# latteine1217/NSFnet

Hardware: AMD Instinct MI355X
Metric: collocation-pt NS-residual evals/sec, Re=2000 6x256 MLP (higher is better)
Workload: dtype bf16x3 (bf16 MFMA, hi/lo split, f32 accumulate)

## Files before the change

include/nsfnet_pinn.h:

```cpp
#ifndef NSFNET_PINN_H
#define NSFNET_PINN_H

#include <stdint.h>

#ifdef __cplusplus
extern "C" {
#endif

typedef struct pinn_net_s* pinn_net_t;
typedef struct pinn_plan_s* pinn_plan_t;

enum {
  PINN_FLD_U = 0, PINN_FLD_V, PINN_FLD_UX, PINN_FLD_UY, PINN_FLD_VX, PINN_FLD_VY,
  PINN_FLD_EQ1, PINN_FLD_EQ2, PINN_FLD_EQ3, PINN_FLD_EQ4, PINN_FLD_P, PINN_FLD_COUNT
};
#define PINN_NLOSS 8

const char* pinn_last_error(void);
int pinn_abi_version(void);

int pinn_net_create(int n_out, int n_hidden_layers, int hidden, pinn_net_t* out);
int pinn_net_destroy(pinn_net_t net);
int pinn_net_set_precision(pinn_net_t net, int prec_fwd, int prec_bwd, int prec_dw);
int64_t pinn_net_num_params(pinn_net_t net);
int64_t pinn_net_prep_floats(pinn_net_t net);
int pinn_net_prepare(pinn_net_t net, const float* params, float* prep, void* stream);

int pinn_plan_create(pinn_net_t net, int64_t n_points, int streams, pinn_plan_t* out);
int pinn_plan_destroy(pinn_plan_t plan);
int64_t pinn_plan_padded_points(pinn_plan_t plan);
int64_t pinn_plan_workspace_bytes(pinn_plan_t plan, int with_backward);
const char* pinn_plan_kernel(pinn_plan_t plan, int which);

int pinn_residual_forward(pinn_plan_t plan, void* ws, const float* prep,
                          const float* x, const float* y, const float* e, const float* w,
                          float* vis_t_minus, float* vis_t_out, float* fields,
                          float Re, float vis_t0, float alpha_evm, float coord_scale,
                          int save, float* loss_sums, void* stream);

int pinn_residual_backward(pinn_plan_t plan, void* ws, const float* prep,
                           const float* x, const float* y, const float* e, const float* w,
                           const float* vis_t, const float* fields, const float* coef_eq4,
                           float Re, float coord_scale, float* ebar_out, void* stream);

int pinn_residual_backward_phases(pinn_plan_t plan, void* ws, const float* prep,
                                  const float* x, const float* y, const float* e, const float* w,
                                  const float* vis_t, const float* fields, const float* coef_eq4,
                                  float Re, float coord_scale, float* ebar_out, int phases, void* stream);

int pinn_residual_forward_backward(pinn_plan_t plan, void* ws, const float* prep,
                                   const float* x, const float* y, const float* e, const float* w,
                                   float* vis_t_minus, float* vis_t_out, float* fields,
                                   const float* coef_eq4, float Re, float vis_t0, float alpha_evm,
                                   float coord_scale, float* loss_sums, float* ebar_out, void* stream);

// ... 94 lines not shown
```

nsfnet_amd/_lib.py:

```python
import ctypes
import os

_HERE = os.path.dirname(os.path.abspath(__file__))
LIB_PATH = os.environ.get("NSFNET_PINN_LIB") or os.path.join(_HERE, "lib", "libnsfnet_pinn.so")

c_void_p, c_int, c_int64, c_float, c_double = ctypes.c_void_p, ctypes.c_int, ctypes.c_int64, ctypes.c_float, ctypes.c_double

SIGNATURES = {
    "pinn_last_error": (ctypes.c_char_p, []),
    "pinn_abi_version": (c_int, []),
    "pinn_net_create": (c_int, [c_int, c_int, c_int, ctypes.POINTER(c_void_p)]),
    "pinn_net_destroy": (c_int, [c_void_p]),
    "pinn_net_set_precision": (c_int, [c_void_p, c_int, c_int, c_int]),
    "pinn_net_num_params": (c_int64, [c_void_p]),
    "pinn_net_prep_floats": (c_int64, [c_void_p]),
    "pinn_net_prepare": (c_int, [c_void_p, c_void_p, c_void_p, c_void_p]),
    "pinn_plan_create": (c_int, [c_void_p, c_int64, c_int, ctypes.POINTER(c_void_p)]),
    "pinn_plan_destroy": (c_int, [c_void_p]),
    "pinn_plan_padded_points": (c_int64, [c_void_p]),
    "pinn_plan_workspace_bytes": (c_int64, [c_void_p, c_int]),
    "pinn_plan_kernel": (ctypes.c_char_p, [c_void_p, c_int]),
    "pinn_residual_forward": (c_int, [c_void_p, c_void_p, c_void_p, c_void_p, c_void_p, c_void_p, c_void_p,
                                      c_void_p, c_void_p, c_void_p, c_float, c_float, c_float, c_float,
                                      c_int, c_void_p, c_void_p]),
    "pinn_residual_backward": (c_int, [c_void_p, c_void_p, c_void_p, c_void_p, c_void_p, c_void_p, c_void_p,
                                       c_void_p, c_void_p, ctypes.POINTER(c_float), c_float, c_float,
                                       c_void_p, c_void_p]),
    "pinn_residual_backward_phases": (c_int, [c_void_p, c_void_p, c_void_p, c_void_p, c_void_p, c_void_p, c_void_p,
                                              c_void_p, c_void_p, ctypes.POINTER(c_float), c_float, c_float,
                                              c_void_p, c_int, c_void_p]),
    "pinn_residual_forward_backward": (c_int, [c_void_p, c_void_p, c_void_p, c_void_p, c_void_p, c_void_p, c_void_p,
                                               c_void_p, c_void_p, c_void_p, ctypes.POINTER(c_float), c_float, c_float,
                                               c_float, c_float, c_void_p, c_void_p, c_void_p]),
    "pinn_value_forward": (c_int, [c_void_p, c_void_p, c_void_p, c_void_p, c_void_p,
                                   ctypes.POINTER(c_void_p), ctypes.POINTER(c_void_p), ctypes.POINTER(c_float),
                                   c_int, c_void_p, c_void_p]),
    "pinn_value_backward": (c_int, [c_void_p, c_void_p, c_void_p, c_void_p, c_void_p, c_void_p, c_void_p]),
    "pinn_grad_reduce": (c_int, [c_void_p, c_int, ctypes.POINTER(c_void_p), ctypes.POINTER(c_void_p),
                                 c_void_p, c_int, c_void_p]),
    "pinn_adam_step": (c_int, [c_void_p, c_void_p, c_void_p, c_void_p, c_int64,
                               c_float, c_float, c_float, c_float, c_int64, c_void_p]),
    "pinn_adam_step_dev": (c_int, [c_void_p, c_void_p, c_void_p, c_void_p, c_int64,
                                   c_float, c_float, c_float, c_float, c_void_p, c_void_p]),
    "pinn_resample_scratch_bytes": (c_int64, [c_int64]),
# ... 75 lines not shown
```

nsfnet_amd/build.py:

```python
import os
import subprocess
import sys
from concurrent.futures import ThreadPoolExecutor

HERE = os.path.dirname(os.path.abspath(__file__))
CSRC = os.path.join(HERE, "csrc")
OBJ = os.path.join(CSRC, "build")
LIBDIR = os.path.join(HERE, "lib")
LIB = os.path.join(LIBDIR, "libnsfnet_pinn.so")
SOURCES = ["fwd.hip", "bwd.hip", "dw.hip", "fwd_bf16.hip", "bwd_bf16.hip", "dw_bf16.hip", "fwd_wide.hip", "bwd_wide.hip", "dw_wide.hip",
           "fwd_bf16_wide.hip", "bwd_bf16_wide.hip", "dw_bf16_wide.hip", "fwd_bf16_pipe.hip", "bwd_bf16_pipe.hip", "fwd_bf16_split.hip", "bwd_bf16_split.hip", "fwdbwd_bf16_split.hip", "fwd_bf16_wsplit.hip", "bwd_bf16_wsplit.hip", "misc.hip", "resample.hip", "lbfgs.hip", "balance.hip", "confgrad.hip", "batch.hip", "rba.hip", "optim.hip", "rwf.hip", "capi.hip"]
HEADERS = ["kernels.h", "layout.h", "spill.h", "spill_io.h", "bf16_util.h", "reduce_util.h", "point_stage.h", "split_phases.h", "wsplit_phases.h", "wave8_bodies.h", "optim.h", "rwf.h", "xwg_fold.h", os.path.join("..", "..", "include", "nsfnet_pinn.h")]
FLAGS = ["-O3", "--offload-arch=gfx950", "-fPIC", "-std=c++17", "-Wall", "-Wno-unused-function"]
_PIPE = ["-fno-slp-vectorize", "-mllvm", "-pragma-unroll-threshold=1000000"]
EXTRA_FLAGS = {"fwd_bf16_pipe.hip": _PIPE, "bwd_bf16_pipe.hip": _PIPE, "fwd_bf16_split.hip": _PIPE, "bwd_bf16_split.hip": _PIPE, "fwdbwd_bf16_split.hip": _PIPE,
               "fwd_bf16_wsplit.hip": _PIPE, "bwd_bf16_wsplit.hip": _PIPE}


def _hipcc():
    for cand in (os.environ.get("HIPCC"), "/opt/rocm/bin/hipcc", "hipcc"):
        if cand and (os.path.isabs(cand) and os.path.exists(cand) or not os.path.isabs(cand)):
            return cand
    return "hipcc"


def _stale(target, deps):
    if not os.path.exists(target):
        return True
    t = os.path.getmtime(target)
    return any(os.path.getmtime(d) > t for d in deps)


def build(force=False, verbose=False):
    os.makedirs(OBJ, exist_ok=True)
    os.makedirs(LIBDIR, exist_ok=True)
# ... 35 lines not shown
```

nsfnet_amd/csrc/balance.hip:

```cpp
#include <cmath>

#include "kernels.h"

namespace {

constexpr int kBlk = 64;
constexpr int kUpdThreads = 256;

__device__ __forceinline__ double nmax(double a, double b) { return (b > a || b != b) ? b : a; }

__device__ __forceinline__ void wave_abs_stats(float v, double& mx, double& sm) {
  mx = fabs((double)v); sm = mx;
#pragma unroll
  for (int off = 32; off > 0; off >>= 1) {
    mx = nmax(mx, __shfl_down(mx, off, 64));
    sm = __dadd_rn(sm, __shfl_down(sm, off, 64));
  }
}

__global__ __launch_bounds__(512) void reduce_terms_kernel(TermReduceArgs a) {
  __shared__ double part[3][8][64];
  const int H = a.H, HP = a.HP, L = a.L;
  const size_t P = flat_total(H, L, a.n_out);
  const int lane = threadIdx.x & 63, w = threadIdx.x >> 6;
  const size_t p = blockIdx.x * (size_t)64 + lane;
  const bool live = p < P;
  const ReduceLoc loc = live ? reduce_locate(p, H, HP, L, a.n_out) : ReduceLoc{-1, -1, 0};
  const size_t SG = sg_total(HP, L);
  int k = 0;
  for (int t = 0; t < 3; ++t) {
    double s = 0.0;
    for (int j = 0; j < a.nsrc[t]; ++j, ++k)
      if (live) s = reduce_source_add(s, a.src[k], loc, HP, SG, w);
    part[t][w][lane] = s;
  }
  __syncthreads();
  if (w != 0) return;
  float vt[3];
  for (int t = 0; t < 3; ++t) {
    float v = 0.f;
    if (a.out[t] && live) {
      double s = part[t][0][lane];
#pragma unroll
      for (int i = 1; i < 8; ++i) s += part[t][i][lane];
      v = (a.acc_mask >> t) & 1 ? a.out[t][p] + (float)s : (float)s;
      a.out[t][p] = v;
    }
    if (a.partials) {
      double mx, sm;
      wave_abs_stats(v, mx, sm);
      if (lane == 0) {
        a.partials[(size_t)blockIdx.x * 6 + 2 * t] = mx;
        a.partials[(size_t)blockIdx.x * 6 + 2 * t + 1] = sm;
      }
    }
    vt[t] = v;
  }
  if (a.gram) wave_gram(vt[0], vt[1], vt[2], lane, a.gram + (size_t)blockIdx.x * 6);
}

__global__ __launch_bounds__(64) void balance_stats_kernel(const float* __restrict__ v0, const float* __restrict__ v1,
                                                           const float* __restrict__ v2, long n,
                                                           double* __restrict__ partials) {
  const long p = blockIdx.x * (long)kBlk + threadIdx.x;
  const float* v[3] = {v0, v1, v2};
  for (int t = 0; t < 3; ++t) {
    double mx, sm;
    wave_abs_stats(v[t] && p < n ? v[t][p] : 0.f, mx, sm);
    if (threadIdx.x == 0) {
      partials[(size_t)blockIdx.x * 6 + 2 * t] = mx;
      partials[(size_t)blockIdx.x * 6 + 2 * t + 1] = sm;
    }
  }
}

__global__ __launch_bounds__(kUpdThreads) void balance_update_kernel(const double* __restrict__ partials, long nblk,
                                                                     long n, int terms, double beta,
                                                                     float* __restrict__ lam, double* record) {
  __shared__ double red[kUpdThreads][6];
  const int tid = threadIdx.x;
  double acc[6] = {0, 0, 0, 0, 0, 0};
// ... 40 lines not shown
}

__global__ void balance_combine_kernel(float* g, const float* gr, const float* __restrict__ gb,
                                       const float* __restrict__ gs, const float* __restrict__ lam, long n) {
  const float lb = lam[0], ls = gs ? lam[1] : 0.f;
  for (long i = blockIdx.x * (long)blockDim.x + threadIdx.x; i < n; i += (long)gridDim.x * blockDim.x) {
    float v = fmaf(lb, gb[i], gr[i]);
    if (gs) v = fmaf(ls, gs[i], v);
    g[i] = v;
  }
}

int status() {
  hipError_t e = hipGetLastError();
  return e == hipSuccess ? 0 : -(int)e;
}

}

long balance_blocks(long n) { return (n + kBlk - 1) / kBlk; }

int launch_reduce_terms(const TermReduceArgs& a, hipStream_t s) {
  size_t P = flat_total(a.H, a.L, a.n_out);
  hipLaunchKernelGGL(reduce_terms_kernel, dim3((unsigned)((P + 63) / 64)), dim3(512), 0, s, a);
  return status();
}

int launch_balance_stats(const float* v0, const float* v1, const float* v2, long n, double* partials, hipStream_t s) {
  hipLaunchKernelGGL(balance_stats_kernel, dim3((unsigned)balance_blocks(n)), dim3(kBlk), 0, s, v0, v1, v2, n, partials);
  return status();
}

int launch_balance_update(const double* partials, long n, int terms, double beta, float* lam, double* record,
                          hipStream_t s) {
  hipLaunchKernelGGL(balance_update_kernel, dim3(1), dim3(kUpdThreads), 0, s, partials, balance_blocks(n), n, terms,
                     beta, lam, record);
  return status();
}

int launch_balance_combine(float* g, const float* gr, const float* gb, const float* gs, const float* lam, long n,
                           hipStream_t s) {
  int blocks = (int)((n + 255) / 256);
  if (blocks > 2048) blocks = 2048;
  hipLaunchKernelGGL(balance_combine_kernel, dim3(blocks), dim3(256), 0, s, g, gr, gb, gs, lam, n);
  return status();
}
```

nsfnet_amd/csrc/capi.hip:

```cpp
#include <cmath>
#include <cstdio>
#include <cstring>
#include <cstdlib>
#include <new>

#include "../../include/nsfnet_pinn.h"
#include "kernels.h"
#include "optim.h"
#include "rwf.h"

static_assert((int)PINN_FLD_COUNT == (int)FLD_COUNT, "field plane enum mismatch");

static thread_local char g_err[512] = "";
static int fail(int code, const char* fmt, const char* a = "", long b = 0) {
  snprintf(g_err, sizeof(g_err), fmt, a, b);
  return code;
}
static int hipfail(int rc, const char* what) {
  if (rc == -1000) return fail(-22, "%s: unsupported hidden width or spill layout (code %ld)", what, (long)rc);
  return fail(rc, "%s: HIP error %ld", what, (long)-rc);
}

struct Switches {
  int sched_f, sched_b;
// ... 352 lines not shown
int pinn_plan_create(pinn_net_t net, int64_t n_points, int streams, pinn_plan_t* out) {
  if (!net || !out) return fail(-22, "pinn_plan_create: null argument%s");
  if (streams != 1 && streams != 4) return fail(-22, "pinn_plan_create: streams must be 1 or 4%s");
  if (n_points < 1 || n_points > (int64_t)1 << 30) return fail(-22, "pinn_plan_create: bad point count %s%ld", "", (long)n_points);
  pinn_plan_s* p = new (std::nothrow) pinn_plan_s;
  if (!p) return fail(-12, "pinn_plan_create: out of host memory%s");
  int rc = resolve_plan(p, *net, (long)n_points, streams, num_cus(), read_switches());
  if (rc) { delete p; return rc; }
  int ndev = 0;
  if (hipGetDeviceCount(&ndev) != hipSuccess) { ndev = 0; (void)hipGetLastError(); }
  if (ndev > 0) {
    rc = configure_plan(p);
    if (rc) { delete p; return hipfail(rc, "pinn_plan_create(kernel attributes)"); }
  }
  *out = p;
  return 0;
}
int pinn_plan_destroy(pinn_plan_t plan) { delete plan; return 0; }
int64_t pinn_plan_padded_points(pinn_plan_t plan) { return plan ? plan->npad : -1; }
const char* pinn_plan_kernel(pinn_plan_t plan, int which) {
  if (!plan || which < 0 || which > 2) return nullptr;
  return plan->role[which == 0 ? ROLE_FWD_SAVE : which == 1 ? ROLE_BWD : ROLE_DW].name;
}
int64_t pinn_plan_workspace_bytes(pinn_plan_t plan, int with_backward) {
  if (!plan) return -1;
  return (int64_t)(with_backward ? plan->bytes_all : plan->bytes_fwd);
}

static int run_loss_sums(const Role& r, const FwdArgs& a, float* loss_sums, hipStream_t s, const char* what) {
  if (!loss_sums) return 0;
  int rc = launch_loss_sums(a.partials, r.grid, loss_sums, s);
  return rc ? hipfail(rc, what) : 0;
}

int pinn_residual_forward(pinn_plan_t plan, void* ws, const float* prep,
                          const float* x, const float* y, const float* e, const float* w,
                          float* vis_t_minus, float* vis_t_out, float* fields,
                          float Re, float vis_t0, float alpha_evm, float coord_scale,
                          int save, float* loss_sums, void* stream) {
  if (!plan || !ws || !prep || !x || !y || !fields) return fail(-22, "pinn_residual_forward: null argument%s");
  if (plan->streams != 4) return fail(-22, "pinn_residual_forward: plan is not a residual (4-stream) plan%s");
  if (!(Re > 0.f)) return fail(-22, "pinn_residual_forward: Re must be > 0%s");
  const FwdArgs a = residual_fwd_args(plan, ws, prep, x, y, e, w, vis_t_minus, vis_t_out, fields, Re, vis_t0, alpha_evm,
                                      coord_scale, save, true);
  const Role& r = plan->role[save ? ROLE_FWD_SAVE : ROLE_FWD];
  int rc = run_fwd(plan, r, a, (hipStream_t)stream);
// ... 493 lines not shown
```

nsfnet_amd/csrc/kernels.h:

```cpp
#pragma once
#include <hip/hip_runtime.h>
#include <type_traits>
#include "layout.h"
#include "spill.h"

typedef float f32x16 __attribute__((ext_vector_type(16)));
typedef float f32x4 __attribute__((ext_vector_type(4)));

#ifdef __HIPCC__
typedef __attribute__((address_space(1))) f32x4 gf32x4;
__device__ __forceinline__ gf32x4* pin_base(const void* q) {
  const unsigned long long b = (unsigned long long)q;
  const unsigned lo = __builtin_amdgcn_readfirstlane((unsigned)b), hi = __builtin_amdgcn_readfirstlane((unsigned)(b >> 32));
  return (gf32x4*)(((unsigned long long)hi << 32) | lo);
}
template <typename... Params, typename... Args>
static int launch_or_configure(void (*kernel)(Params...), dim3 grid, dim3 block, size_t lds, hipStream_t s, int configure,
                               const Args&... args) {
  if (configure)
    return -(int)hipFuncSetAttribute(reinterpret_cast<const void*>(kernel), hipFuncAttributeMaxDynamicSharedMemorySize, PINN_LDS_MAX);
  hipLaunchKernelGGL(kernel, grid, block, lds, s, args...);
  return -(int)hipGetLastError();
}
template <class F>
// ... 64 lines not shown

struct ReduceLoc { int sgi; int layer; size_t slab_off; };
__device__ __forceinline__ ReduceLoc reduce_locate(size_t p, int H, int HP, int L, int n_out) {
  ReduceLoc r{-1, -1, 0};
  if (p < (size_t)2 * H) {
    int o = (int)(p / 2), j = (int)(p % 2);
    r.sgi = (j == 0 ? sg_w0x(HP, L) : sg_w0y(HP, L)) + o;
  } else if (p < (size_t)3 * H) {
    r.sgi = sg_db(HP, 0) + (int)(p - 2 * H);
  } else if (p < flat_w(H, L)) {
    size_t rel = p - (size_t)3 * H;
    size_t per = (size_t)H * H + H;
    int l = 1 + (int)(rel / per);
    size_t q = rel % per;
    if (q < (size_t)H * H) { r.layer = l; r.slab_off = (q / H) * HP + (q % H); }
    else r.sgi = sg_db(HP, l) + (int)(q - (size_t)H * H);
  } else {
    size_t q = p - flat_w(H, L);
    if (q < (size_t)n_out * H) r.sgi = sg_wout(HP, L) + (int)(q / H) * HP + (int)(q % H);
    else r.sgi = sg_bout(HP, L) + (int)(q - (size_t)n_out * H);
  }
  return r;
}
__device__ __forceinline__ double reduce_source_add(double s, const ReduceSrc& src, const ReduceLoc& loc, int HP,
                                                    size_t SG, int w) {
  const float* base; size_t stride; int n;
  if (loc.layer >= 0) { base = src.slabs + (size_t)(loc.layer - 1) * src.groups * HP * HP + loc.slab_off; stride = (size_t)HP * HP; n = src.groups; }
  else { base = src.sg + loc.sgi; stride = SG; n = src.nwg; }
  int g = w;
  for (; g + 24 < n; g += 32) {
    float v0 = base[(size_t)g * stride], v1 = base[(size_t)(g + 8) * stride];
    float v2 = base[(size_t)(g + 16) * stride], v3 = base[(size_t)(g + 24) * stride];
    s += (double)v0; s += (double)v1; s += (double)v2; s += (double)v3;
  }
  for (; g < n; g += 8) s += (double)base[(size_t)g * stride];
  return s;
}

struct TermReduceArgs {
  ReduceSrc src[4]; int nsrc[3];
  int H, HP, L, n_out;
  float* out[3]; int acc_mask;
  double* partials;
  double* gram;
};

__device__ __forceinline__ void wave_gram(float r, float b, float s, int lane, double* __restrict__ out) {
  const double dr = r, db = b, ds = s;
  double q[6] = {__dmul_rn(dr, dr), __dmul_rn(db, db), __dmul_rn(ds, ds),
                 __dmul_rn(dr, db), __dmul_rn(dr, ds), __dmul_rn(db, ds)};
#pragma unroll
  for (int off = 32; off > 0; off >>= 1) {
#pragma unroll
    for (int c = 0; c < 6; ++c) q[c] = __dadd_rn(q[c], __shfl_down(q[c], off, 64));
  }
  if (lane == 0) {
#pragma unroll
    for (int c = 0; c < 6; ++c) out[c] = q[c];
  }
// ... 97 lines not shown
```

nsfnet_amd/csrc/misc.hip:

```cpp
#include "kernels.h"

__device__ __forceinline__ unsigned short f2bf_rne(float x) {
  return __builtin_bit_cast(unsigned short, (__bf16)x);
}

__device__ __forceinline__ unsigned short bf16_frag_elem(const float* W, int H, int HP, bool tr, int pos, int lo_part) {
  int j = pos & 7, lane = (pos >> 3) & 63, ws = pos >> 9;
  int KS = HP / 16, s = ws % KS, w = ws / KS;
  int k = 16 * s + 8 * (lane >> 5) + j, o = 32 * w + (lane & 31);
  float v = 0.f;
  if (o < H && k < H) v = tr ? W[(size_t)k * H + o] : W[(size_t)o * H + k];
  unsigned short hi = f2bf_rne(v);
  if (!lo_part) return hi;
  return f2bf_rne(v - __uint_as_float(((unsigned)hi) << 16));
}

__global__ void prep_kernel(const float* __restrict__ params, float* __restrict__ prep,
                            int H, int HP, int L, int n_out, int prec_fwd, int prec_bwd) {
  const size_t total = prep_total(HP, L);
  for (size_t idx = blockIdx.x * (size_t)blockDim.x + threadIdx.x; idx < total;
       idx += (size_t)gridDim.x * blockDim.x) {
    float v = 0.f;
    if (idx < (size_t)3 * HP) {
      int which = (int)(idx / HP), o = (int)(idx % HP);
      if (o < H) v = which == 0 ? params[flat_w(H, 0) + 2 * o] : which == 1 ? params[flat_w(H, 0) + 2 * o + 1]
                                                                            : params[flat_b(H, 0, L, n_out) + o];
    } else if (idx < prep_wout(HP, L)) {
      size_t rel = idx - (size_t)3 * HP;
      int l = 1 + (int)(rel / prep_layer_stride(HP));
      size_t q = rel % prep_layer_stride(HP);
      const float* W = params + flat_w(H, l);
      if (q < (size_t)2 * HP * HP) {
        bool tr = q >= (size_t)HP * HP;
        size_t f = tr ? q - (size_t)HP * HP : q;
        if ((tr ? prec_bwd : prec_fwd) != 0) {
          int e0 = (int)(2 * f), half = HP * HP;
          unsigned short b0 = bf16_frag_elem(W, H, HP, tr, e0 % half, e0 / half);
          unsigned short b1 = bf16_frag_elem(W, H, HP, tr, (e0 + 1) % half, (e0 + 1) / half);
          prep[idx] = __uint_as_float((unsigned)b0 | ((unsigned)b1 << 16));
          continue;
        }
        int e = (int)(f & 3), lane = (int)((f >> 2) & 63);
        int wq = (int)(f >> 8);
        int qq = wq % (HP / 8), w = wq / (HP / 8);
        int k = 2 * (4 * qq + e) + (lane >> 5), o = 32 * w + (lane & 31);
        if (o < H && k < H) v = tr ? W[(size_t)k * H + o] : W[(size_t)o * H + k];
      } else {
        int o = (int)(q - (size_t)2 * HP * HP);
        if (o < H) v = params[flat_b(H, l, L, n_out) + o];
      }
    } else if (idx < prep_bout(HP, L)) {
      size_t q = idx - prep_wout(HP, L);
      int c = (int)(q / HP), k = (int)(q % HP);
      if (c < n_out && k < H) v = params[flat_w(H, L) + (size_t)c * H + k];
    } else {
      int c = (int)(idx - prep_bout(HP, L));
      if (c < n_out) v = params[flat_b(H, L, L, n_out) + c];
    }
    prep[idx] = v;
  }
}

int launch_prep(const float* params, float* prep, int H, int HP, int L, int n_out, int prec_fwd, int prec_bwd,
                hipStream_t s) {
  size_t total = prep_total(HP, L);
  int blocks = (int)((total + 255) / 256);
  if (blocks > 4096) blocks = 4096;
  hipLaunchKernelGGL(prep_kernel, dim3(blocks), dim3(256), 0, s, params, prep, H, HP, L, n_out, prec_fwd, prec_bwd);
  hipError_t e = hipGetLastError();
  return e == hipSuccess ? 0 : -(int)e;
}

__global__ __launch_bounds__(512) void reduce_kernel(ReduceArgs a) {
  __shared__ double part[8][64];
  const int H = a.H, HP = a.HP, L = a.L;
  const size_t P = flat_total(H, L, a.n_out);
  const int lane = threadIdx.x & 63, w = threadIdx.x >> 6;
  const size_t p = blockIdx.x * (size_t)64 + lane;
  const bool live = p < P;
  const ReduceLoc loc = live ? reduce_locate(p, H, HP, L, a.n_out) : ReduceLoc{-1, -1, 0};
  double s = 0.0;
  if (live) {
    const size_t SG = sg_total(HP, L);
    for (int k = 0; k < a.nsrc; ++k) s = reduce_source_add(s, a.src[k], loc, HP, SG, w);
  }
  part[w][lane] = s;
  __syncthreads();
  if (w == 0 && live) {
    double t = part[0][lane];
#pragma unroll
    for (int i = 1; i < 8; ++i) t += part[i][lane];
    if (a.accumulate) a.grads[p] += (float)t; else a.grads[p] = (float)t;
  }
}

int launch_reduce(const ReduceArgs& a, hipStream_t s) {
  size_t P = flat_total(a.H, a.L, a.n_out);
  hipLaunchKernelGGL(reduce_kernel, dim3((unsigned)((P + 63) / 64)), dim3(512), 0, s, a);
  hipError_t e = hipGetLastError();
  return e == hipSuccess ? 0 : -(int)e;
}

__global__ __launch_bounds__(256) void loss_sums_kernel(const float* __restrict__ partials, int nparts, float* __restrict__ out) {
  __shared__ double part[32][PINN_NLOSS];
  const int k = threadIdx.x % PINN_NLOSS, j = threadIdx.x / PINN_NLOSS;
  double s = 0.0;
  for (int i = j; i < nparts; i += 32) s += (double)partials[(size_t)i * PINN_NLOSS + k];
  part[j][k] = s;
  __syncthreads();
  if (threadIdx.x < PINN_NLOSS) {
    double t = part[0][k];
    for (int i = 1; i < 32; ++i) t += part[i][k];
    out[k] = (float)t;
  }
}

int launch_loss_sums(const float* partials, int nparts, float* out, hipStream_t s) {
  static_assert(PINN_NLOSS * 32 == 256, "loss_sums_kernel layout");
  hipLaunchKernelGGL(loss_sums_kernel, dim3(1), dim3(256), 0, s, partials, nparts, out);
  hipError_t e = hipGetLastError();
  return e == hipSuccess ? 0 : -(int)e;
}

__global__ void adam_kernel(float* __restrict__ p, const float* __restrict__ g, float* __restrict__ m,
                            float* __restrict__ v, long n, float step_size, float b1, float b2, float eps,
                            float bc2_sqrt) {
  for (long i = blockIdx.x * (long)blockDim.x + threadIdx.x; i < n; i += (long)gridDim.x * blockDim.x) {
    float gi = g[i];
    float mi = m[i] + (gi - m[i]) * (1.f - b1);
    float vi = v[i] * b2 + (1.f - b2) * gi * gi;
    float denom = sqrtf(vi) / bc2_sqrt + eps;
    p[i] = p[i] - step_size * (mi / denom);
    m[i] = mi; v[i] = vi;
  }
}

__global__ void adam_dev_kernel(float* __restrict__ p, const float* __restrict__ g, float* __restrict__ m,
                                float* __restrict__ v, long n, float lr, float b1, float b2, float eps,
                                long long* step_counter) {
  const double t = (double)(__atomic_load_n(step_counter, __ATOMIC_RELAXED) + 1);
  const double bc1 = 1.0 - pow((double)b1, t), bc2 = 1.0 - pow((double)b2, t);
  const float step_size = (float)((double)lr / bc1), bc2_sqrt = (float)sqrt(bc2);
  for (long i = blockIdx.x * (long)blockDim.x + threadIdx.x; i < n; i += (long)gridDim.x * blockDim.x) {
    float gi = g[i];
    float mi = m[i] + (gi - m[i]) * (1.f - b1);
    float vi = v[i] * b2 + (1.f - b2) * gi * gi;
    float denom = sqrtf(vi) / bc2_sqrt + eps;
    p[i] = p[i] - step_size * (mi / denom);
    m[i] = mi; v[i] = vi;
  }
  __syncthreads();
  if (threadIdx.x == 0) {
    unsigned long long* ticket = reinterpret_cast<unsigned long long*>(step_counter + 1);
    __threadfence();
    if (atomicAdd(ticket, 1ull) == (unsigned long long)gridDim.x - 1) {
      *ticket = 0;
      step_counter[0] = step_counter[0] + 1;
    }
  }
}

int launch_adam_dev(float* p, const float* g, float* m, float* v, long n, float lr, float b1, float b2,
                    float eps, long long* step_counter, hipStream_t s) {
  if (n <= 0) return 0;
  int blocks = (int)((n + 255) / 256);
  if (blocks > 2048) blocks = 2048;
  hipLaunchKernelGGL(adam_dev_kernel, dim3(blocks), dim3(256), 0, s, p, g, m, v, n, lr, b1, b2, eps, step_counter);
  hipError_t e = hipGetLastError();
  return e == hipSuccess ? 0 : -(int)e;
}

int launch_adam(float* p, const float* g, float* m, float* v, long n, float step_size, float b1, float b2,
                float eps, float bc2_sqrt, hipStream_t s) {
  if (n <= 0) return 0;
  int blocks = (int)((n + 255) / 256);
  if (blocks > 2048) blocks = 2048;
  hipLaunchKernelGGL(adam_kernel, dim3(blocks), dim3(256), 0, s, p, g, m, v, n, step_size, b1, b2, eps, bc2_sqrt);
  hipError_t e = hipGetLastError();
  return e == hipSuccess ? 0 : -(int)e;
}
```

nsfnet_amd/csrc/optim.hip:

```cpp
#include "optim.h"
#include "xwg_fold.h"

namespace {

constexpr int kThreads = 256;
constexpr int kPer = 4;
constexpr int kTile = kThreads * kPer;
constexpr int kMaxBlocksVec = 256;
constexpr int kTicket = 1, kPart = 8;
constexpr int kScratchDoubles = kPart + 2 * kMaxBlocksVec;

__host__ __device__ inline long blocks_of(long n) {
  const long b = (n + kTile - 1) / kTile;
  return b < kMaxBlocksVec ? b : kMaxBlocksVec;
}

__global__ __launch_bounds__(kThreads) void grad_sqnorm_kernel(const float* __restrict__ g0, long n0,
                                                               const float* __restrict__ g1, long n1, double* scratch) {
  __shared__ double red[kThreads / 64];
  __shared__ double tree[kThreads];
  __shared__ int flag;
  const long nb0 = blocks_of(n0);
  const bool second = (long)blockIdx.x >= nb0;
  const float* __restrict__ g = second ? g1 : g0;
// ... 22 lines not shown
    double t = red[0];
    for (int i = 1; i < kThreads / 64; ++i) t += red[i];
    put(scratch + kPart + blockIdx.x, t);
  }
  if (!last_block(scratch + kTicket, &flag)) return;
  double f = 0.0;
  for (int k = threadIdx.x; k < (int)gridDim.x; k += kThreads) f += get(scratch + kPart + k);
  tree[threadIdx.x] = f;
  __syncthreads();
  for (int half = kThreads / 2; half > 0; half >>= 1) {
    if (threadIdx.x < half) tree[threadIdx.x] += tree[threadIdx.x + half];
    __syncthreads();
  }
  if (threadIdx.x == 0) scratch[0] = tree[0];
}

__device__ __forceinline__ float scaled(float g, float coef) {
#pragma clang fp contract(off)
  const float r = g * coef;
  return r;
}

template <bool CLIP>
__global__ void adam_sched_kernel(AdamSchedArgs a) {
  const long long e = __atomic_load_n(a.epoch, __ATOMIC_RELAXED);
  const float lr = (float)lr_schedule_value(a.sched, a.lr0, e);
  double norm = 0.0;
  float coef = 1.f;
  if (CLIP) {
    norm = sqrt(a.sq[0]);
    const double c = a.max_norm / (norm + 1e-6);
    coef = (float)(c > 1.0 ? 1.0 : c);
  }
  const float b1 = a.b1, b2 = a.b2, eps = a.eps;
  float* __restrict__ p = a.p;
  const float* __restrict__ g = a.g;
  float* __restrict__ m = a.m;
  float* __restrict__ v = a.v;
  const double t = (double)(__atomic_load_n(a.step_counter, __ATOMIC_RELAXED) + 1);
  const double bc1 = 1.0 - pow((double)b1, t), bc2 = 1.0 - pow((double)b2, t);
  const float step_size = (float)((double)lr / bc1), bc2_sqrt = (float)sqrt(bc2);
  for (long i = blockIdx.x * (long)blockDim.x + threadIdx.x; i < a.n; i += (long)gridDim.x * blockDim.x) {
    float gi = CLIP ? scaled(g[i], coef) : g[i];
    float mi = m[i] + (gi - m[i]) * (1.f - b1);
    float vi = v[i] * b2 + (1.f - b2) * gi * gi;
    float denom = sqrtf(vi) / bc2_sqrt + eps;
    p[i] = p[i] - step_size * (mi / denom);
    m[i] = mi; v[i] = vi;
  }
  __syncthreads();
  if (threadIdx.x == 0) {
    unsigned long long* ticket = reinterpret_cast<unsigned long long*>(a.step_counter + 1);
    __threadfence();
    if (atomicAdd(ticket, 1ull) == (unsigned long long)gridDim.x - 1) {
      *ticket = 0;
      a.step_counter[0] = a.step_counter[0] + 1;
      a.record[0] = (double)e;
      a.record[1] = (double)lr;
      a.record[2] = norm;
      a.record[3] = (double)coef;
      if (a.advance) {
        a.epoch[0] = e + 1;
        if (coef < 1.f) a.record[4] += 1.0;
        a.record[5] += 1.0;
      }
    }
  }
}

int status() {
  hipError_t e = hipGetLastError();
  return e == hipSuccess ? 0 : -(int)e;
}

}

size_t grad_sqnorm_scratch_bytes() { return (size_t)kScratchDoubles * sizeof(double); }

int launch_grad_sqnorm(const float* g0, long n0, const float* g1, long n1, double* scratch, hipStream_t s) {
  const long blocks = blocks_of(n0) + (n1 > 0 ? blocks_of(n1) : 0);
  hipLaunchKernelGGL(grad_sqnorm_kernel, dim3((unsigned)blocks), dim3(kThreads), 0, s, g0, n0, g1, n1, scratch);
  return status();
}

int launch_adam_sched(const AdamSchedArgs& a, hipStream_t s) {
  if (a.n <= 0) return 0;
  int blocks = (int)((a.n + 255) / 256);
  if (blocks > 2048) blocks = 2048;
  if (a.sq) hipLaunchKernelGGL(adam_sched_kernel<true>, dim3(blocks), dim3(256), 0, s, a);
  else hipLaunchKernelGGL(adam_sched_kernel<false>, dim3(blocks), dim3(256), 0, s, a);
  return status();
}
```

Before: 43.60 million.

## Vectorize gradient reduction, Adam updates, and pow2 index math in prep kernel

The gradient reduce kernels now give each lane four consecutive parameters and use float4 loads from the per-group slabs, with a deeper 8-way unroll. Adam is factored into a shared helper that uses float4 sweeps, 1024-thread blocks capped at 64 blocks, and bias-correction scalars computed once per block. The prep kernel swaps division and modulo for shifts and masks when HP is a power of two and uses 32-bit indices. Together these target memory throughput and integer overhead in the per-step optimizer and reduce phases, at the cost of more code paths and a fallback for misaligned runs.

```diff
diff --git a/include/nsfnet_pinn.h b/include/nsfnet_pinn.h
--- a/include/nsfnet_pinn.h
+++ b/include/nsfnet_pinn.h
@@ -31,6 +31,7 @@
 int64_t pinn_plan_padded_points(pinn_plan_t plan);
 int64_t pinn_plan_workspace_bytes(pinn_plan_t plan, int with_backward);
 const char* pinn_plan_kernel(pinn_plan_t plan, int which);
+int pinn_plan_reduce_layout(pinn_plan_t plan, int64_t* out4);
 
 int pinn_residual_forward(pinn_plan_t plan, void* ws, const float* prep,
                           const float* x, const float* y, const float* e, const float* w,
diff --git a/nsfnet_amd/_lib.py b/nsfnet_amd/_lib.py
--- a/nsfnet_amd/_lib.py
+++ b/nsfnet_amd/_lib.py
@@ -20,6 +20,7 @@
     "pinn_plan_padded_points": (c_int64, [c_void_p]),
     "pinn_plan_workspace_bytes": (c_int64, [c_void_p, c_int]),
     "pinn_plan_kernel": (ctypes.c_char_p, [c_void_p, c_int]),
+    "pinn_plan_reduce_layout": (c_int, [c_void_p, ctypes.POINTER(c_int64)]),
     "pinn_residual_forward": (c_int, [c_void_p, c_void_p, c_void_p, c_void_p, c_void_p, c_void_p, c_void_p,
                                       c_void_p, c_void_p, c_void_p, c_float, c_float, c_float, c_float,
                                       c_int, c_void_p, c_void_p]),
diff --git a/nsfnet_amd/build.py b/nsfnet_amd/build.py
--- a/nsfnet_amd/build.py
+++ b/nsfnet_amd/build.py
@@ -10,7 +10,7 @@
 LIB = os.path.join(LIBDIR, "libnsfnet_pinn.so")
 SOURCES = ["fwd.hip", "bwd.hip", "dw.hip", "fwd_bf16.hip", "bwd_bf16.hip", "dw_bf16.hip", "fwd_wide.hip", "bwd_wide.hip", "dw_wide.hip",
            "fwd_bf16_wide.hip", "bwd_bf16_wide.hip", "dw_bf16_wide.hip", "fwd_bf16_pipe.hip", "bwd_bf16_pipe.hip", "fwd_bf16_split.hip", "bwd_bf16_split.hip", "fwdbwd_bf16_split.hip", "fwd_bf16_wsplit.hip", "bwd_bf16_wsplit.hip", "misc.hip", "resample.hip", "lbfgs.hip", "balance.hip", "confgrad.hip", "batch.hip", "rba.hip", "optim.hip", "rwf.hip", "capi.hip"]
-HEADERS = ["kernels.h", "layout.h", "spill.h", "spill_io.h", "bf16_util.h", "reduce_util.h", "point_stage.h", "split_phases.h", "wsplit_phases.h", "wave8_bodies.h", "optim.h", "rwf.h", "xwg_fold.h", os.path.join("..", "..", "include", "nsfnet_pinn.h")]
+HEADERS = ["kernels.h", "layout.h", "spill.h", "spill_io.h", "bf16_util.h", "reduce_util.h", "point_stage.h", "split_phases.h", "wsplit_phases.h", "wave8_bodies.h", "optim.h", "rwf.h", "xwg_fold.h", "adam_update.h", os.path.join("..", "..", "include", "nsfnet_pinn.h")]
 FLAGS = ["-O3", "--offload-arch=gfx950", "-fPIC", "-std=c++17", "-Wall", "-Wno-unused-function"]
 _PIPE = ["-fno-slp-vectorize", "-mllvm", "-pragma-unroll-threshold=1000000"]
 EXTRA_FLAGS = {"fwd_bf16_pipe.hip": _PIPE, "bwd_bf16_pipe.hip": _PIPE, "fwd_bf16_split.hip": _PIPE, "bwd_bf16_split.hip": _PIPE, "fwdbwd_bf16_split.hip": _PIPE,
diff --git a/nsfnet_amd/csrc/adam_update.h b/nsfnet_amd/csrc/adam_update.h
--- /dev/null
+++ b/nsfnet_amd/csrc/adam_update.h
@@ -0,0 +1,57 @@
+#pragma once
+#include <hip/hip_runtime.h>
+#include <stdint.h>
+
+constexpr int kAdamThreads = 1024;
+constexpr int kAdamMaxBlocks = 64;
+static inline int adam_blocks(long n) {
+  const long b = (n + 4L * kAdamThreads - 1) / (4L * kAdamThreads);
+  return (int)(b < 1 ? 1 : b > kAdamMaxBlocks ? kAdamMaxBlocks : b);
+}
+
+struct AdamScalars { float step_size, bc2_sqrt; };
+__device__ __forceinline__ AdamScalars adam_scalars(float lr, float b1, float b2, const long long* step_counter) {
+  __shared__ float sc[2];
+  if (threadIdx.x == 0) {
+    const double t = (double)(__atomic_load_n(step_counter, __ATOMIC_RELAXED) + 1);
+    const double bc1 = 1.0 - pow((double)b1, t), bc2 = 1.0 - pow((double)b2, t);
+    sc[0] = (float)((double)lr / bc1);
+    sc[1] = (float)sqrt(bc2);
+  }
+  __syncthreads();
+  return AdamScalars{sc[0], sc[1]};
+}
+
+__device__ __forceinline__ void adam_update(float& p, float g, float& m, float& v, float step_size, float b1, float b2,
+                                            float eps, float bc2_sqrt) {
+#pragma clang fp contract(off)
+  const float mi = m + (g - m) * (1.f - b1);
+  const float vi = v * b2 + (1.f - b2) * g * g;
+  const float denom = sqrtf(vi) / bc2_sqrt + eps;
+  p = __builtin_fmaf(-(mi / denom), step_size, p);
+  m = mi; v = vi;
+}
+
+template <class G>
+__device__ __forceinline__ void adam_sweep(float* __restrict__ p, const float* __restrict__ g, float* __restrict__ m,
+                                           float* __restrict__ v, long n, AdamScalars sc, float b1, float b2, float eps,
+                                           G grad) {
+  const long tid = blockIdx.x * (long)blockDim.x + threadIdx.x, stride = (long)gridDim.x * blockDim.x;
+  const bool aligned = ((reinterpret_cast<uintptr_t>(p) | reinterpret_cast<uintptr_t>(g) | reinterpret_cast<uintptr_t>(m) |
+                         reinterpret_cast<uintptr_t>(v)) & 15) == 0;
+  const long nq = aligned ? n / 4 : 0;
+  for (long i = tid; i < nq; i += stride) {
+    float4 pi = reinterpret_cast<float4*>(p)[i], mi = reinterpret_cast<float4*>(m)[i], vi = reinterpret_cast<float4*>(v)[i];
+    const float4 gi = reinterpret_cast<const float4*>(g)[i];
+    adam_update(pi.x, grad(gi.x), mi.x, vi.x, sc.step_size, b1, b2, eps, sc.bc2_sqrt);
+    adam_update(pi.y, grad(gi.y), mi.y, vi.y, sc.step_size, b1, b2, eps, sc.bc2_sqrt);
+    adam_update(pi.z, grad(gi.z), mi.z, vi.z, sc.step_size, b1, b2, eps, sc.bc2_sqrt);
+    adam_update(pi.w, grad(gi.w), mi.w, vi.w, sc.step_size, b1, b2, eps, sc.bc2_sqrt);
+    reinterpret_cast<float4*>(p)[i] = pi; reinterpret_cast<float4*>(m)[i] = mi; reinterpret_cast<float4*>(v)[i] = vi;
+  }
+  for (long i = 4 * nq + tid; i < n; i += stride) {
+    float pi = p[i], mi = m[i], vi = v[i];
+    adam_update(pi, grad(g[i]), mi, vi, sc.step_size, b1, b2, eps, sc.bc2_sqrt);
+    p[i] = pi; m[i] = mi; v[i] = vi;
+  }
+}
diff --git a/nsfnet_amd/csrc/balance.hip b/nsfnet_amd/csrc/balance.hip
--- a/nsfnet_amd/csrc/balance.hip
+++ b/nsfnet_amd/csrc/balance.hip
@@ -19,30 +19,31 @@
 }
 
 __global__ __launch_bounds__(512) void reduce_terms_kernel(TermReduceArgs a) {
-  __shared__ double part[3][8][64];
+  __shared__ double part[3][8][kReduceBlock];
   const int H = a.H, HP = a.HP, L = a.L;
   const size_t P = flat_total(H, L, a.n_out);
   const int lane = threadIdx.x & 63, w = threadIdx.x >> 6;
-  const size_t p = blockIdx.x * (size_t)64 + lane;
-  const bool live = p < P;
-  const ReduceLoc loc = live ? reduce_locate(p, H, HP, L, a.n_out) : ReduceLoc{-1, -1, 0};
+  const size_t p0 = blockIdx.x * (size_t)kReduceBlock;
+  const ReduceLoc4 q = reduce_locate4(p0 + 4 * lane, P, H, HP, L, a.n_out);
   const size_t SG = sg_total(HP, L);
   int k = 0;
   for (int t = 0; t < 3; ++t) {
-    double s = 0.0;
-    for (int j = 0; j < a.nsrc[t]; ++j, ++k)
-      if (live) s = reduce_source_add(s, a.src[k], loc, HP, SG, w);
-    part[t][w][lane] = s;
+    double s[4] = {0.0, 0.0, 0.0, 0.0};
+    for (int j = 0; j < a.nsrc[t]; ++j, ++k) reduce_source_add4(s, a.src[k], q, HP, SG, w);
+#pragma unroll
+    for (int j = 0; j < 4; ++j) part[t][w][4 * lane + j] = s[j];
   }
   __syncthreads();
-  if (w != 0) return;
+  const size_t blk = (size_t)blockIdx.x * (kReduceBlock / kBlk) + w, p = blk * kBlk + lane;
+  if (w >= kReduceBlock / kBlk || blk * kBlk >= P) return;
+  const bool live = p < P;
   float vt[3];
   for (int t = 0; t < 3; ++t) {
     float v = 0.f;
     if (a.out[t] && live) {
-      double s = part[t][0][lane];
+      double s = part[t][0][threadIdx.x];
 #pragma unroll
-      for (int i = 1; i < 8; ++i) s += part[t][i][lane];
+      for (int i = 1; i < 8; ++i) s += part[t][i][threadIdx.x];
       v = (a.acc_mask >> t) & 1 ? a.out[t][p] + (float)s : (float)s;
       a.out[t][p] = v;
     }
@@ -50,13 +51,13 @@
       double mx, sm;
       wave_abs_stats(v, mx, sm);
       if (lane == 0) {
-        a.partials[(size_t)blockIdx.x * 6 + 2 * t] = mx;
-        a.partials[(size_t)blockIdx.x * 6 + 2 * t + 1] = sm;
+        a.partials[blk * 6 + 2 * t] = mx;
+        a.partials[blk * 6 + 2 * t + 1] = sm;
       }
     }
     vt[t] = v;
   }
-  if (a.gram) wave_gram(vt[0], vt[1], vt[2], lane, a.gram + (size_t)blockIdx.x * 6);
+  if (a.gram) wave_gram(vt[0], vt[1], vt[2], lane, a.gram + blk * 6);
 }
 
 __global__ __launch_bounds__(64) void balance_stats_kernel(const float* __restrict__ v0, const float* __restrict__ v1,
@@ -143,7 +144,7 @@
 
 int launch_reduce_terms(const TermReduceArgs& a, hipStream_t s) {
   size_t P = flat_total(a.H, a.L, a.n_out);
-  hipLaunchKernelGGL(reduce_terms_kernel, dim3((unsigned)((P + 63) / 64)), dim3(512), 0, s, a);
+  hipLaunchKernelGGL(reduce_terms_kernel, dim3((unsigned)((P + kReduceBlock - 1) / kReduceBlock)), dim3(512), 0, s, a);
   return status();
 }
 
diff --git a/nsfnet_amd/csrc/capi.hip b/nsfnet_amd/csrc/capi.hip
--- a/nsfnet_amd/csrc/capi.hip
+++ b/nsfnet_amd/csrc/capi.hip
@@ -398,6 +398,12 @@
   if (!plan || which < 0 || which > 2) return nullptr;
   return plan->role[which == 0 ? ROLE_FWD_SAVE : which == 1 ? ROLE_BWD : ROLE_DW].name;
 }
+int pinn_plan_reduce_layout(pinn_plan_t plan, int64_t* out4) {
+  if (!plan || !out4) return fail(-22, "pinn_plan_reduce_layout: null argument%s");
+  out4[0] = (int64_t)plan->off_sg; out4[1] = plan->role[ROLE_BWD].grid;
+  out4[2] = (int64_t)plan->off_slabs; out4[3] = plan->groups;
+  return 0;
+}
 int64_t pinn_plan_workspace_bytes(pinn_plan_t plan, int with_backward) {
   if (!plan) return -1;
   return (int64_t)(with_backward ? plan->bytes_all : plan->bytes_fwd);
diff --git a/nsfnet_amd/csrc/kernels.h b/nsfnet_amd/csrc/kernels.h
--- a/nsfnet_amd/csrc/kernels.h
+++ b/nsfnet_amd/csrc/kernels.h
@@ -110,19 +110,70 @@
   }
   return r;
 }
+__device__ __forceinline__ const float* reduce_source_base(const ReduceSrc& src, const ReduceLoc& loc, int HP, size_t SG,
+                                                           size_t& stride, int& n) {
+  if (loc.layer >= 0) { stride = (size_t)HP * HP; n = src.groups; return src.slabs + (size_t)(loc.layer - 1) * src.groups * HP * HP + loc.slab_off; }
+  stride = SG; n = src.nwg;
+  return src.sg + loc.sgi;
+}
 __device__ __forceinline__ double reduce_source_add(double s, const ReduceSrc& src, const ReduceLoc& loc, int HP,
                                                     size_t SG, int w) {
-  const float* base; size_t stride; int n;
-  if (loc.layer >= 0) { base = src.slabs + (size_t)(loc.layer - 1) * src.groups * HP * HP + loc.slab_off; stride = (size_t)HP * HP; n = src.groups; }
-  else { base = src.sg + loc.sgi; stride = SG; n = src.nwg; }
+  size_t stride; int n;
+  const float* base = reduce_source_base(src, loc, HP, SG, stride, n);
   int g = w;
-  for (; g + 24 < n; g += 32) {
-    float v0 = base[(size_t)g * stride], v1 = base[(size_t)(g + 8) * stride];
-    float v2 = base[(size_t)(g + 16) * stride], v3 = base[(size_t)(g + 24) * stride];
-    s += (double)v0; s += (double)v1; s += (double)v2; s += (double)v3;
+  for (; g + 56 < n; g += 64) {
+    float v[8];
+#pragma unroll
+    for (int i = 0; i < 8; ++i) v[i] = base[(size_t)(g + 8 * i) * stride];
+#pragma unroll
+    for (int i = 0; i < 8; ++i) s += (double)v[i];
   }
   for (; g < n; g += 8) s += (double)base[(size_t)g * stride];
   return s;
+}
+
+constexpr int kReduceBlock = 256;
+struct ReduceLoc4 { ReduceLoc loc[4]; bool run; };
+__device__ __forceinline__ ReduceLoc4 reduce_locate4(size_t p0, size_t P, int H, int HP, int L, int n_out) {
+  ReduceLoc4 q;
+#pragma unroll
+  for (int j = 0; j < 4; ++j) q.loc[j] = p0 + j < P ? reduce_locate(p0 + j, H, HP, L, n_out) : ReduceLoc{-1, -1, 0};
+  const bool slab = q.loc[0].layer >= 0;
+  bool run = p0 + 3 < P && (slab ? q.loc[0].slab_off % 4 == 0 : q.loc[0].sgi % 4 == 0);
+#pragma unroll
+  for (int j = 1; j < 4; ++j)
+    run = run && q.loc[j].layer == q.loc[0].layer &&
+          (slab ? q.loc[j].slab_off == q.loc[0].slab_off + j : q.loc[j].sgi == q.loc[0].sgi + j);
+  q.run = run;
+  return q;
+}
+__device__ __forceinline__ void reduce_source_add4(double (&s)[4], const ReduceSrc& src, const ReduceLoc4& q, int HP,
+                                                   size_t SG, int w) {
+  const bool aligned = ((reinterpret_cast<uintptr_t>(src.slabs) | reinterpret_cast<uintptr_t>(src.sg)) & 15) == 0;
+  if (q.run && aligned) {
+    size_t stride; int n;
+    const float* base = reduce_source_base(src, q.loc[0], HP, SG, stride, n);
+    int g = w;
+    for (; g + 56 < n; g += 64) {
+      f32x4 v[8];
+#pragma unroll
+      for (int i = 0; i < 8; ++i) v[i] = *reinterpret_cast<const f32x4*>(base + (size_t)(g + 8 * i) * stride);
+#pragma unroll
+      for (int i = 0; i < 8; ++i) {
+#pragma unroll
+        for (int j = 0; j < 4; ++j) s[j] += (double)v[i][j];
+      }
+    }
+    for (; g < n; g += 8) {
+      const f32x4 v = *reinterpret_cast<const f32x4*>(base + (size_t)g * stride);
+#pragma unroll
+      for (int j = 0; j < 4; ++j) s[j] += (double)v[j];
+    }
+  } else {
+#pragma unroll
+    for (int j = 0; j < 4; ++j)
+      if (q.loc[j].layer >= 0 || q.loc[j].sgi >= 0) s[j] = reduce_source_add(s[j], src, q.loc[j], HP, SG, w);
+  }
 }
 
 struct TermReduceArgs {
diff --git a/nsfnet_amd/csrc/misc.hip b/nsfnet_amd/csrc/misc.hip
--- a/nsfnet_amd/csrc/misc.hip
+++ b/nsfnet_amd/csrc/misc.hip
@@ -1,12 +1,18 @@
 #include "kernels.h"
+#include "adam_update.h"
 
 __device__ __forceinline__ unsigned short f2bf_rne(float x) {
   return __builtin_bit_cast(unsigned short, (__bf16)x);
 }
 
-__device__ __forceinline__ unsigned short bf16_frag_elem(const float* W, int H, int HP, bool tr, int pos, int lo_part) {
-  int j = pos & 7, lane = (pos >> 3) & 63, ws = pos >> 9;
-  int KS = HP / 16, s = ws % KS, w = ws / KS;
+template <bool POW2> __device__ __forceinline__ unsigned quo(unsigned x, unsigned d, int sh) { return POW2 ? x >> sh : x / d; }
+template <bool POW2> __device__ __forceinline__ unsigned rem(unsigned x, unsigned d, int sh) { return POW2 ? x & (d - 1) : x % d; }
+
+template <bool POW2>
+__device__ __forceinline__ unsigned short bf16_frag_elem(const float* W, int H, int HP, int shp, bool tr, unsigned pos, int lo_part) {
+  int j = pos & 7, lane = (pos >> 3) & 63;
+  unsigned ws = pos >> 9;
+  int s = (int)rem<POW2>(ws, HP / 16, shp - 4), w = (int)quo<POW2>(ws, HP / 16, shp - 4);
   int k = 16 * s + 8 * (lane >> 5) + j, o = 32 * w + (lane & 31);
   float v = 0.f;
   if (o < H && k < H) v = tr ? W[(size_t)k * H + o] : W[(size_t)o * H + k];
@@ -15,46 +21,48 @@
   return f2bf_rne(v - __uint_as_float(((unsigned)hi) << 16));
 }
 
+template <bool POW2>
 __global__ void prep_kernel(const float* __restrict__ params, float* __restrict__ prep,
-                            int H, int HP, int L, int n_out, int prec_fwd, int prec_bwd) {
-  const size_t total = prep_total(HP, L);
-  for (size_t idx = blockIdx.x * (size_t)blockDim.x + threadIdx.x; idx < total;
-       idx += (size_t)gridDim.x * blockDim.x) {
+                            int H, int HP, int shp, int L, int n_out, int prec_fwd, int prec_bwd) {
+  const unsigned total = (unsigned)prep_total(HP, L), wout = (unsigned)prep_wout(HP, L), bout = (unsigned)prep_bout(HP, L);
+  const unsigned lstride = (unsigned)prep_layer_stride(HP), half = (unsigned)HP * HP;
+  for (unsigned idx = blockIdx.x * blockDim.x + threadIdx.x; idx < total; idx += gridDim.x * blockDim.x) {
     float v = 0.f;
-    if (idx < (size_t)3 * HP) {
-      int which = (int)(idx / HP), o = (int)(idx % HP);
+    if (idx < 3u * HP) {
+      int which = (int)quo<POW2>(idx, HP, shp), o = (int)rem<POW2>(idx, HP, shp);
       if (o < H) v = which == 0 ? params[flat_w(H, 0) + 2 * o] : which == 1 ? params[flat_w(H, 0) + 2 * o + 1]
                                                                             : params[flat_b(H, 0, L, n_out) + o];
-    } else if (idx < prep_wout(HP, L)) {
-      size_t rel = idx - (size_t)3 * HP;
-      int l = 1 + (int)(rel / prep_layer_stride(HP));
-      size_t q = rel % prep_layer_stride(HP);
+    } else if (idx < wout) {
+      unsigned rel = idx - 3u * HP;
+      unsigned lq = rel / lstride;
+      int l = 1 + (int)lq;
+      unsigned q = rel - lq * lstride;
       const float* W = params + flat_w(H, l);
-      if (q < (size_t)2 * HP * HP) {
-        bool tr = q >= (size_t)HP * HP;
-        size_t f = tr ? q - (size_t)HP * HP : q;
+      if (q < 2 * half) {
+        bool tr = q >= half;
+        unsigned f = tr ? q - half : q;
         if ((tr ? prec_bwd : prec_fwd) != 0) {
-          int e0 = (int)(2 * f), half = HP * HP;
-          unsigned short b0 = bf16_frag_elem(W, H, HP, tr, e0 % half, e0 / half);
-          unsigned short b1 = bf16_frag_elem(W, H, HP, tr, (e0 + 1) % half, (e0 + 1) / half);
+          unsigned e0 = 2 * f;
+          unsigned short b0 = bf16_frag_elem<POW2>(W, H, HP, shp, tr, rem<POW2>(e0, half, 2 * shp), (int)quo<POW2>(e0, half, 2 * shp));
+          unsigned short b1 = bf16_frag_elem<POW2>(W, H, HP, shp, tr, rem<POW2>(e0 + 1, half, 2 * shp), (int)quo<POW2>(e0 + 1, half, 2 * shp));
           prep[idx] = __uint_as_float((unsigned)b0 | ((unsigned)b1 << 16));
           continue;
         }
         int e = (int)(f & 3), lane = (int)((f >> 2) & 63);
-        int wq = (int)(f >> 8);
-        int qq = wq % (HP / 8), w = wq / (HP / 8);
+        unsigned wq = f >> 8;
+        int qq = (int)rem<POW2>(wq, HP / 8, shp - 3), w = (int)quo<POW2>(wq, HP / 8, shp - 3);
         int k = 2 * (4 * qq + e) + (lane >> 5), o = 32 * w + (lane & 31);
         if (o < H && k < H) v = tr ? W[(size_t)k * H + o] : W[(size_t)o * H + k];
       } else {
-        int o = (int)(q - (size_t)2 * HP * HP);
+        int o = (int)(q - 2 * half);
         if (o < H) v = params[flat_b(H, l, L, n_out) + o];
       }
-    } else if (idx < prep_bout(HP, L)) {
-      size_t q = idx - prep_wout(HP, L);
-      int c = (int)(q / HP), k = (int)(q % HP);
+    } else if (idx < bout) {
+      unsigned q = idx - wout;
+      int c = (int)quo<POW2>(q, HP, shp), k = (int)rem<POW2>(q, HP, shp);
       if (c < n_out && k < H) v = params[flat_w(H, L) + (size_t)c * H + k];
     } else {
-      int c = (int)(idx - prep_bout(HP, L));
+      int c = (int)(idx - bout);
       if (c < n_out) v = params[flat_b(H, L, L, n_out) + c];
     }
     prep[idx] = v;
@@ -64,39 +72,44 @@
 int launch_prep(const float* params, float* prep, int H, int HP, int L, int n_out, int prec_fwd, int prec_bwd,
                 hipStream_t s) {
   size_t total = prep_total(HP, L);
+  if (total >= (size_t)1 << 31) return -(int)hipErrorInvalidValue;
   int blocks = (int)((total + 255) / 256);
   if (blocks > 4096) blocks = 4096;
-  hipLaunchKernelGGL(prep_kernel, dim3(blocks), dim3(256), 0, s, params, prep, H, HP, L, n_out, prec_fwd, prec_bwd);
+  int shp = 0;
+  while ((1 << shp) < HP) ++shp;
+  if ((1 << shp) == HP && HP >= 32)
+    hipLaunchKernelGGL(prep_kernel<true>, dim3(blocks), dim3(256), 0, s, params, prep, H, HP, shp, L, n_out, prec_fwd, prec_bwd);
+  else
+    hipLaunchKernelGGL(prep_kernel<false>, dim3(blocks), dim3(256), 0, s, params, prep, H, HP, shp, L, n_out, prec_fwd, prec_bwd);
   hipError_t e = hipGetLastError();
   return e == hipSuccess ? 0 : -(int)e;
 }
 
 __global__ __launch_bounds__(512) void reduce_kernel(ReduceArgs a) {
-  __shared__ double part[8][64];
+  __shared__ double part[8][kReduceBlock];
   const int H = a.H, HP = a.HP, L = a.L;
   const size_t P = flat_total(H, L, a.n_out);
   const int lane = threadIdx.x & 63, w = threadIdx.x >> 6;
-  const size_t p = blockIdx.x * (size_t)64 + lane;
-  const bool live = p < P;
-  const ReduceLoc loc = live ? reduce_locate(p, H, HP, L, a.n_out) : ReduceLoc{-1, -1, 0};
-  double s = 0.0;
-  if (live) {
-    const size_t SG = sg_total(HP, L);
-    for (int k = 0; k < a.nsrc; ++k) s = reduce_source_add(s, a.src[k], loc, HP, SG, w);
-  }
-  part[w][lane] = s;
+  const size_t p0 = blockIdx.x * (size_t)kReduceBlock;
+  const ReduceLoc4 q = reduce_locate4(p0 + 4 * lane, P, H, HP, L, a.n_out);
+  const size_t SG = sg_total(HP, L);
+  double s[4] = {0.0, 0.0, 0.0, 0.0};
+  for (int k = 0; k < a.nsrc; ++k) reduce_source_add4(s, a.src[k], q, HP, SG, w);
+#pragma unroll
+  for (int j = 0; j < 4; ++j) part[w][4 * lane + j] = s[j];
   __syncthreads();
-  if (w == 0 && live) {
-    double t = part[0][lane];
+  const size_t p = p0 + threadIdx.x;
+  if (threadIdx.x < kReduceBlock && p < P) {
+    double t = part[0][threadIdx.x];
 #pragma unroll
-    for (int i = 1; i < 8; ++i) t += part[i][lane];
+    for (int i = 1; i < 8; ++i) t += part[i][threadIdx.x];
     if (a.accumulate) a.grads[p] += (float)t; else a.grads[p] = (float)t;
   }
 }
 
 int launch_reduce(const ReduceArgs& a, hipStream_t s) {
   size_t P = flat_total(a.H, a.L, a.n_out);
-  hipLaunchKernelGGL(reduce_kernel, dim3((unsigned)((P + 63) / 64)), dim3(512), 0, s, a);
+  hipLaunchKernelGGL(reduce_kernel, dim3((unsigned)((P + kReduceBlock - 1) / kReduceBlock)), dim3(512), 0, s, a);
   hipError_t e = hipGetLastError();
   return e == hipSuccess ? 0 : -(int)e;
 }
@@ -135,20 +148,12 @@
   }
 }
 
-__global__ void adam_dev_kernel(float* __restrict__ p, const float* __restrict__ g, float* __restrict__ m,
-                                float* __restrict__ v, long n, float lr, float b1, float b2, float eps,
-                                long long* step_counter) {
-  const double t = (double)(__atomic_load_n(step_counter, __ATOMIC_RELAXED) + 1);
-  const double bc1 = 1.0 - pow((double)b1, t), bc2 = 1.0 - pow((double)b2, t);
-  const float step_size = (float)((double)lr / bc1), bc2_sqrt = (float)sqrt(bc2);
-  for (long i = blockIdx.x * (long)blockDim.x + threadIdx.x; i < n; i += (long)gridDim.x * blockDim.x) {
-    float gi = g[i];
-    float mi = m[i] + (gi - m[i]) * (1.f - b1);
-    float vi = v[i] * b2 + (1.f - b2) * gi * gi;
-    float denom = sqrtf(vi) / bc2_sqrt + eps;
-    p[i] = p[i] - step_size * (mi / denom);
-    m[i] = mi; v[i] = vi;
-  }
+__global__ __launch_bounds__(kAdamThreads) void adam_dev_kernel(float* __restrict__ p, const float* __restrict__ g,
+                                                                float* __restrict__ m, float* __restrict__ v, long n,
+                                                                float lr, float b1, float b2, float eps,
+                                                                long long* step_counter) {
+  const AdamScalars sc = adam_scalars(lr, b1, b2, step_counter);
+  adam_sweep(p, g, m, v, n, sc, b1, b2, eps, [](float gi) { return gi; });
   __syncthreads();
   if (threadIdx.x == 0) {
     unsigned long long* ticket = reinterpret_cast<unsigned long long*>(step_counter + 1);
@@ -163,9 +168,8 @@
 int launch_adam_dev(float* p, const float* g, float* m, float* v, long n, float lr, float b1, float b2,
                     float eps, long long* step_counter, hipStream_t s) {
   if (n <= 0) return 0;
-  int blocks = (int)((n + 255) / 256);
-  if (blocks > 2048) blocks = 2048;
-  hipLaunchKernelGGL(adam_dev_kernel, dim3(blocks), dim3(256), 0, s, p, g, m, v, n, lr, b1, b2, eps, step_counter);
+  hipLaunchKernelGGL(adam_dev_kernel, dim3(adam_blocks(n)), dim3(kAdamThreads), 0, s, p, g, m, v, n, lr, b1, b2, eps,
+                     step_counter);
   hipError_t e = hipGetLastError();
   return e == hipSuccess ? 0 : -(int)e;
 }
diff --git a/nsfnet_amd/csrc/optim.hip b/nsfnet_amd/csrc/optim.hip
--- a/nsfnet_amd/csrc/optim.hip
+++ b/nsfnet_amd/csrc/optim.hip
@@ -1,5 +1,6 @@
 #include "optim.h"
 #include "xwg_fold.h"
+#include "adam_update.h"
 
 namespace {
 
@@ -68,7 +69,7 @@
 }
 
 template <bool CLIP>
-__global__ void adam_sched_kernel(AdamSchedArgs a) {
+__global__ __launch_bounds__(kAdamThreads) void adam_sched_kernel(AdamSchedArgs a) {
   const long long e = __atomic_load_n(a.epoch, __ATOMIC_RELAXED);
   const float lr = (float)lr_schedule_value(a.sched, a.lr0, e);
   double norm = 0.0;
@@ -83,17 +84,8 @@
   const float* __restrict__ g = a.g;
   float* __restrict__ m = a.m;
   float* __restrict__ v = a.v;
-  const double t = (double)(__atomic_load_n(a.step_counter, __ATOMIC_RELAXED) + 1);
-  const double bc1 = 1.0 - pow((double)b1, t), bc2 = 1.0 - pow((double)b2, t);
-  const float step_size = (float)((double)lr / bc1), bc2_sqrt = (float)sqrt(bc2);
-  for (long i = blockIdx.x * (long)blockDim.x + threadIdx.x; i < a.n; i += (long)gridDim.x * blockDim.x) {
-    float gi = CLIP ? scaled(g[i], coef) : g[i];
-    float mi = m[i] + (gi - m[i]) * (1.f - b1);
-    float vi = v[i] * b2 + (1.f - b2) * gi * gi;
-    float denom = sqrtf(vi) / bc2_sqrt + eps;
-    p[i] = p[i] - step_size * (mi / denom);
-    m[i] = mi; v[i] = vi;
-  }
+  const AdamScalars sc = adam_scalars(lr, b1, b2, a.step_counter);
+  adam_sweep(p, g, m, v, a.n, sc, b1, b2, eps, [coef](float gi) { return CLIP ? scaled(gi, coef) : gi; });
   __syncthreads();
   if (threadIdx.x == 0) {
     unsigned long long* ticket = reinterpret_cast<unsigned long long*>(a.step_counter + 1);
@@ -131,9 +123,8 @@
 
 int launch_adam_sched(const AdamSchedArgs& a, hipStream_t s) {
   if (a.n <= 0) return 0;
-  int blocks = (int)((a.n + 255) / 256);
-  if (blocks > 2048) blocks = 2048;
-  if (a.sq) hipLaunchKernelGGL(adam_sched_kernel<true>, dim3(blocks), dim3(256), 0, s, a);
-  else hipLaunchKernelGGL(adam_sched_kernel<false>, dim3(blocks), dim3(256), 0, s, a);
+  const int blocks = adam_blocks(a.n);
+  if (a.sq) hipLaunchKernelGGL(adam_sched_kernel<true>, dim3(blocks), dim3(kAdamThreads), 0, s, a);
+  else hipLaunchKernelGGL(adam_sched_kernel<false>, dim3(blocks), dim3(kAdamThreads), 0, s, a);
   return status();
 }
```

New measurement: 43.74 million (median of 6 runs). No clear change (+0.3%).
